# h3poteto/aws-global-accelerator-controller

Measured on NVIDIA H100. Metric: objects reconciled/sec at 10^6 Service+Ingress; change-set bit-exact vs Go ref, higher is better.
Workload: dtype u8/u32 (bytes and indices)

## Files before the change

### aws-global-accelerator-controller_b200/csrc/gar_engine.cu

```cuda

#include <cuda_runtime.h>
#include <unistd.h>

#include <cstdio>
#include <cstdlib>
#include <cstring>
#include <atomic>
#include <exception>
#include <functional>
#include <mutex>
#include <thread>
#include <string>
#include <vector>
#include <type_traits>
#include <utility>

#include "gar_pipeline.h"
#include "gar_shard.h"
#include "gar_delta.h"

#define GAR_VERSION_STRING "garecon 0.1.0 (sm_90a)"


template <class F>
// ... 97 lines not shown
template <class... Fs>
struct FPack;
template <>
struct FPack<> {
  __device__ __forceinline__ void call(int, u32) const {}
};
template <class F, class... R>
struct FPack<F, R...> {
  F f;
  FPack<R...> rest;
  FPack(const F &f_, const R &...r) : f(f_), rest(r...) {}
  __device__ __forceinline__ void call(int k, u32 i) const {
    if (k == 0) f(i);
    else rest.call(k - 1, i);
  }
};
constexpr int MULTI_MAX = 8;
struct MultiRanges {
  u32 blk_end[MULTI_MAX], n[MULTI_MAX];
  int count;
};
template <class P>
__global__ void __launch_bounds__(256) k_for_each_multi(const __grid_constant__ P pack, const __grid_constant__ MultiRanges r) {
  int k = 0;
  while (k + 1 < r.count && blockIdx.x >= r.blk_end[k]) k++;
  u32 i = (blockIdx.x - (k ? r.blk_end[k - 1] : 0u)) * blockDim.x + threadIdx.x;
  if (i < r.n[k]) pack.call(k, i);
}

template <class F> struct MinBlocks { static constexpr int value = 2; };
template <> struct MinBlocks<FGaObj> { static constexpr int value = 4; };
template <> struct MinBlocks<FR53Pair> { static constexpr int value = 6; };
template <> struct MinBlocks<FR53Prepare> { static constexpr int value = 6; };

__global__ void k_fill32(u32 *p, u32 v, size_t n) {
  size_t i = (size_t)blockIdx.x * blockDim.x + threadIdx.x;
  size_t stride = (size_t)gridDim.x * blockDim.x;
  for (; i < n; i += stride) p[i] = v;
}

constexpr int SCAN_THREADS = 256;
constexpr int SCAN_ITEMS = 8;
constexpr int SCAN_TILE = SCAN_THREADS * SCAN_ITEMS;

__device__ __forceinline__ u32 warp_incl_scan(u32 v) {
  const unsigned lane = threadIdx.x & 31;
#pragma unroll
  for (int d = 1; d < 32; d <<= 1) {
    u32 t = __shfl_up_sync(0xffffffffu, v, d);
    if (lane >= (unsigned)d) v += t;
  }
  return v;
}
__device__ __forceinline__ u32 block_excl_scan(u32 v, u32 *total) {
  __shared__ u32 wsum[SCAN_THREADS / 32];
  __shared__ u32 wtot;
  const unsigned lane = threadIdx.x & 31, w = threadIdx.x >> 5;
  u32 inc = warp_incl_scan(v);
  if (lane == 31) wsum[w] = inc;
  __syncthreads();
  if (w == 0) {
    u32 s = lane < SCAN_THREADS / 32 ? wsum[lane] : 0;
    u32 si = warp_incl_scan(s);
    if (lane < SCAN_THREADS / 32) wsum[lane] = si - s;
    if (lane == SCAN_THREADS / 32 - 1) wtot = si;
  }
// ... 1551 lines not shown
```

### aws-global-accelerator-controller_b200/csrc/gar_pipeline.h

```cpp
#pragma once

#include <stdio.h>
#include <stdlib.h>

#include <initializer_list>

#include "gar_rows.h"

#if defined(__CUDA_ARCH__)
#define GAR_ATOMIC_ADD(p, v) atomicAdd((p), (v))
#else
#define GAR_ATOMIC_ADD(p, v) (*(p) += (v))
#endif


enum Slot {
  S_DERIVED, S_OFLAGS, S_OKEY_HASH, S_STAGE_GA, S_STAGE_R53, S_ANN_R53, S_ANN_NAME, S_ANN_TAGS, S_ANN_LISTEN, S_DPORT_BEGIN, S_DPORTS,
  S_TOK_CODE, S_TOK_NAME, S_TOK_REGION,
  S_ACC_FLAGS, S_ACC_OWNER_KEY, S_ACC_OWNER, S_ACC_THOST, S_ACC_MANAGED, S_ACC_OWNER_HASH, S_ACC_THOST_HASH, S_REC_NAME_HASH, S_VAL_KEY_HASH,
  S_REC_ZONE, S_VAL_REC, S_VAL_CLS, S_VAL_KEY, S_VAL_ORPHAN, S_VAL_LINK, S_ACC_DIGEST,
  S_R53_MODE, S_R53_ACC, S_R53_ACC_DNS, S_PAIR_BEGIN, S_PAIR_OBJ, S_PAIR_HN, S_PAIR_CODE, S_PAIR_ZONE, S_PAIR_REC,
  S_IX_LB, S_IX_OWNER = S_IX_LB + 3, S_IX_THOST = S_IX_OWNER + 3, S_IX_ZONE = S_IX_THOST + 3, S_IX_VAL = S_IX_ZONE + 3,
  S_IX_ALIAS = S_IX_VAL + 3, S_IX_OBJ = S_IX_ALIAS + 3, S_IX_OVN = S_IX_OBJ + 3,
  S_SORT_KEYS = S_IX_OVN + 3, S_SORT_VALS, S_SORT_KEYS_ALT, S_SORT_VALS_ALT, S_SORT_TAGS,
  S_COUNTS, S_STATUS_GA, S_STATUS_R53, S_OPS, S_ERRFLAG, S_IX_EG, S_IX_EG_ENT, S_IX_EG_PAD,
  S_VAL_OBJ, S_ACC_OBJ, S_OBJ_CANON, S_OWN_BEGIN, S_OWN_FILL, S_OWN_ENT, S_OWN_MULTI,
  S_IXA_BEGIN, S_IXA_FILL, S_IXA_ENT, S_IXA_MULTI, S_OVN_FILL, S_OVN_MULTI, S_LB_HASH, S_REC_FLAGS,
  S_NSLOTS
};


struct FClassify {
  DevTables T;
  Work W;
  u32 *derived_public;
  u8 *oflags;
  u32 *errflag;
  GAR_HD void operator()(u32 i) const {
    classify_object(T, W, i);
    W.obj_canon[i] = i;
    u32 dv = W.derived[i];
    if (dv & OBJ_KEY_BAD) GAR_ATOMIC_ADD(errflag, 1u);
    derived_public[i] = dv & 0xFFu;
  }
};
struct FTokenise {
  DevTables T;
  Work W;
  static constexpr int kStageCols = 1;
  static constexpr u32 kStageBytes = 24 * 1024;
  static constexpr bool kStageByDefault = true;
  GAR_HD void operator()(u32 i) const { tokenise_hostname(T, W, i); }
  GAR_HD const u8 *stage_slab(int) const { return T.o.slab; }
  GAR_HD bool stage_window(int, u32 r0, u32 r1, u64 *lo, u64 *hi) const {
    gar_str a = T.o.lbi_hostname[r0], b = T.o.lbi_hostname[r1 - 1];
    *lo = GAR_STR_OFF(a);
    *hi = GAR_STR_OFF(b) + GAR_STR_LEN(b);
    return true;
  }
  template <class View>
  GAR_HD void run(u32 i, const View &view) const { tokenise_hostname_at(T, W, i, view(0, T.o.lbi_hostname[i])); }
};
struct FDigestAccel {
  DevTables T;
  Work W;
  GAR_HD void operator()(u32 i) const { digest_accelerator(T, W, i); }
};
struct FExpand {
  const u32 *begin;
  u32 nparents;
  u32 *parent_of;
  GAR_HD void operator()(u32 c) const {
    u32 lo = 0, hi = nparents;
    while (hi - lo > 1) {
      u32 mid = (lo + hi) >> 1;
      if (begin[mid] <= c) lo = mid;
      else hi = mid;
    }
    parent_of[c] = lo;
  }
};
constexpr u32 REC_INLINE_VALUES = 32;
constexpr u32 REC_HUGE_VALUES = 4096;
struct DirectView {
  const u8 *slab;
  GAR_HD Str operator()(int, gar_str r) const { return mkstr(slab, r); }
};
struct FPrepareRecord {
  DevTables T;
  Work W;
  u32 *big, *huge;
  static constexpr int kStageCols = 2;
  static constexpr u32 kStageBytes = 16 * 1024;
  static constexpr bool kStageByDefault = true;
  GAR_HD const u8 *stage_slab(int) const { return T.a.slab; }
  GAR_HD bool stage_window(int c, u32 r0, u32 r1, u64 *lo, u64 *hi) const {
    if (c == 0) {
      gar_str a = T.a.rec_name[r0], b = T.a.rec_name[r1 - 1];
      *lo = GAR_STR_OFF(a);
// ... 744 lines not shown
      be.for_each("idx_place", nrows, FIdxPlace{keys, cursor, tmp, ent, nb});
      be.for_each("idx_order", nb, FIdxOrder{begin, ent, overflow, canon});
    } else if (nrows) {
      u32 *keys2 = (u32 *)be.ensure(S_SORT_KEYS_ALT, sizeof(u32) * (size_t)(nrows + 1));
      u32 *vals2 = (u32 *)be.ensure(S_SORT_VALS_ALT, sizeof(u32) * (size_t)(nrows + 1));
      be.sort_pairs(keys, vals, keys2, vals2, nrows, ilog2(nb) + 1);
      be.for_each("idx_gather", nrows, FIdxGather{vals, begin + nb, tmp, ent});
      if (canon.canon) be.for_each("idx_order", nb, FIdxCanon{begin, ent, canon});
    }
    return HashIdx{begin, ent, nb - 1};
  }

  bool prepared = false;
  u64 n_dports = 0;
  u32 *errflag = nullptr;

  u32 acc_guest_from = 0xFFFFFFFFu;
  u32 sharded = 0;
  bool orphan_sweep = true;
  bool allow_empty_cache = false;

  void alloc_obj_work() {
    const u32 n = T.o.n_objects, nlbi = T.o.n_lbi;
    W.derived = (u32 *)be.ensure(S_DERIVED, 4 * (size_t)(n + 1));
    W.okey_hash = (u64 *)be.ensure(S_OKEY_HASH, 8 * (size_t)(n + 1));
    W.ann_r53 = (gar_str *)be.ensure(S_ANN_R53, 8 * (size_t)(n + 1));
    W.ann_name = (gar_str *)be.ensure(S_ANN_NAME, 8 * (size_t)(n + 1));
    W.ann_tags = (gar_str *)be.ensure(S_ANN_TAGS, 8 * (size_t)(n + 1));
    W.ann_listen = (gar_str *)be.ensure(S_ANN_LISTEN, 8 * (size_t)(n + 1));
    W.dport_begin = (u32 *)be.out_dport_begin(n);
    W.tok_code = (u8 *)be.out_tok_code(nlbi);
    W.tok_name = (gar_str *)be.out_tok_name(nlbi);
    W.tok_region = (gar_str *)be.out_tok_region(nlbi);
    W.r53_mode = (u8 *)be.ensure(S_R53_MODE, (size_t)n + 1);
    W.r53_acc = (u32 *)be.ensure(S_R53_ACC, 4 * (size_t)(n + 1));
    W.r53_acc_dns = (gar_str *)be.ensure(S_R53_ACC_DNS, 8 * (size_t)(n + 1));
    W.obj_canon = (u32 *)be.ensure(S_OBJ_CANON, 4 * (size_t)(n + 1));
  }
  CanonHook canon_hook(u32 b0, u32 b1) const { return CanonHook{W.obj_canon, T.o.slab, b0, b1}; }
  void alloc_work() {
    const u32 nacc = T.a.n_accels, nrec = T.a.n_records, nval = T.a.n_values;
    alloc_obj_work();
    W.acc_flags = (u32 *)be.ensure(S_ACC_FLAGS, 4 * (size_t)(nacc + 1));
    W.acc_owner_key = (gar_str *)be.ensure(S_ACC_OWNER_KEY, 8 * (size_t)(nacc + 1));
    W.acc_owner = (gar_str *)be.ensure(S_ACC_OWNER, 8 * (size_t)(nacc + 1));
    W.acc_thost = (gar_str *)be.ensure(S_ACC_THOST, 8 * (size_t)(nacc + 1));
    W.acc_managed = (gar_str *)be.ensure(S_ACC_MANAGED, 8 * (size_t)(nacc + 1));
    W.acc_owner_hash = (u64 *)be.ensure(S_ACC_OWNER_HASH, 8 * (size_t)(nacc + 1));
    W.acc_thost_hash = (u64 *)be.ensure(S_ACC_THOST_HASH, 8 * (size_t)(nacc + 1));
    W.rec_name_hash = (u64 *)be.ensure(S_REC_NAME_HASH, 8 * (size_t)(nrec + 1));
    W.val_key_hash = (u64 *)be.ensure(S_VAL_KEY_HASH, 8 * (size_t)(nval + 1));
    W.rec_zone = (u32 *)be.ensure(S_REC_ZONE, 4 * (size_t)(nrec + 1));
    W.val_rec = (u32 *)be.ensure(S_VAL_REC, 4 * (size_t)(nval + 1));
    W.val_cls = (u8 *)be.ensure(S_VAL_CLS, nval + 1);
    W.val_key = (gar_str *)be.ensure(S_VAL_KEY, 8 * (size_t)(nval + 1));
    W.val_orphan = (u8 *)be.ensure(S_VAL_ORPHAN, nval + 1);
    W.val_obj = (u32 *)be.ensure(S_VAL_OBJ, 4 * (size_t)(nval + 1));
    W.acc_obj = (u32 *)be.ensure(S_ACC_OBJ, 4 * (size_t)(nacc + 1));
    W.val_link = (ValLink *)be.ensure(S_VAL_LINK, sizeof(ValLink) * (size_t)(nval + 1));
    W.acc_digest = (AccDigest *)be.ensure(S_ACC_DIGEST, sizeof(AccDigest) * (size_t)(nacc + 1));
    W.lb_hash = (u64 *)be.ensure(S_LB_HASH, 8 * (size_t)(T.a.n_lbs + 1));
    W.rec_flags = (u8 *)be.ensure(S_REC_FLAGS, (size_t)nrec + 1);
    for (int k = 0; k < IX_N; k++) W.hist[k] = IxHist{nullptr, 0};
    W.pair_cap = 0;
    W.dport_cap = 0;
    errflag = (u32 *)be.ensure(S_ERRFLAG, 256);
// ... 144 lines not shown
    arm_group_a(1u << IX_ALIAS);
    stage1();
    finish_group_a();
  }
  void prepare_directory() {
    alloc_work();
    arm_group_a((1u << IX_LB) | (1u << IX_THOST));
    if (T.o.n_lbi) be.for_each("tokenise_hostnames", T.o.n_lbi, FTokenise{T, W});
    if (T.a.n_accels) be.for_each("digest_accelerators", T.a.n_accels, FDigestAccel{T, W});
    if (T.a.n_lbs) be.for_each("hash_load_balancers", T.a.n_lbs, FLbHash{T, W});
    finish_group_a();
  }

  u32 dport_cap = 0, pair_cap = 0;
  u64 ops_cap = 0;
  bool tiny_caps = false;
  int prepare() {
    const u32 n = T.o.n_objects, nacc = T.a.n_accels, nzone = T.a.n_zones, nrec = T.a.n_records;
    alloc_work();
    if (!force_radix) arm_group_a((1u << IX_LB) | (1u << IX_THOST) | (1u << IX_ZONE) | (1u << IX_ALIAS) | (1u << IX_OBJ));
    stage1();
    listen_ports();

    u32 *overflow = errflag + FW_IDX_OVERFLOW;
    if (!force_radix) {
      finish_group_a();
    } else {
      W.ix_lb = build_index(S_IX_LB, T.a.n_lbs, 1, FRowLb{T, W}, overflow, true);
      W.ix_thost = build_index(S_IX_THOST, nacc, 1, FRowThost{T, W}, overflow, true);
      W.ix_zone = build_index(S_IX_ZONE, nzone, 1, FRowZone{T}, overflow, true);
      W.ix_alias = build_index(S_IX_ALIAS, nrec, 2, FRowAlias{T, W}, overflow, true);
      W.ix_obj = build_index(S_IX_OBJ, n, 1, FRowObj{T, W}, overflow, true, canon_hook(0, 0xFFFFFFFFu));
    }
    resolve_owners(true);
    obj_stale = false;
    owner_indexes = false;
    return GAR_OK;
  }
  void listen_ports() {
    const u32 n = T.o.n_objects;
    be.fill32(W.dport_begin, 0, (size_t)n + 1);
    if (n) be.for_each("listen_ports_count", n, FJsonCount{T, W});
    be.exclusive_scan(W.dport_begin, n + 1);
    be.for_each("gather_header", 1, FGatherHeader{W.dport_begin + n, errflag});
    if (dport_cap < n / 2 + 1024 && !(tiny_caps && dport_cap)) dport_cap = tiny_caps ? 1 : n / 2 + 1024;
    W.dport_cap = dport_cap;
    W.dports = (i32 *)be.out_dports(dport_cap);
    if (n) be.for_each("listen_ports_write", n, FJsonWrite{T, W});
  }

  bool obj_stale = false, owners_stale = false;
  void prepare_objects() {
    const u32 n = T.o.n_objects, nlbi = T.o.n_lbi;
    alloc_obj_work();
    be.fill32(errflag, 0, FW_WORDS);
    W.hist[IX_OBJ] = IxHist{nullptr, 0};
    u32 *derived_public = (u32 *)be.out_derived(n);
    if (n) be.for_each("classify_objects", n, FClassify{T, W, derived_public, nullptr, errflag});
    if (nlbi) be.for_each_staged("tokenise_hostnames", nlbi, FTokenise{T, W});
    listen_ports();
    W.ix_obj = build_index(S_IX_OBJ, n, 1, FRowObj{T, W}, errflag + FW_IDX_OVERFLOW, force_radix, canon_hook(0, 0xFFFFFFFFu));
    obj_stale = false;
    owners_stale = true;
  }
  int index_objects() {
    for (int attempt = 0; attempt < 2; attempt++) {
      if (!prepared) prepare();
      else if (obj_stale) prepare_objects();
      prepared = true;
      u32 fl[FW_WORDS];
      be.download(fl, errflag, sizeof(fl));
      if (fl[FW_BAD_KEYS]) return GAR_E_INVALID;
      if (fl[FW_IDX_OVERFLOW] && !force_radix) {
        force_radix = true;
        prepared = false;
        continue;
      }
      return GAR_OK;
    }
    return GAR_E_STATE;
  }

  u64 n_pairs = 0;
  void r53_relational(u32 slots, const u32 *rows, u32 *st_r53) {
    W.pair_begin = (u32 *)be.ensure(S_PAIR_BEGIN, 4 * (size_t)(slots + 2));
    be.fill32(W.pair_begin, 0, (size_t)slots + 1);
    if (slots) be.for_each_warp("r53_prepare", slots, FR53Prepare{T, W, st_r53, rows});
    be.exclusive_scan(W.pair_begin, slots + 1);
    if (pair_cap < slots + slots / 2 + 1024 && !(tiny_caps && pair_cap)) pair_cap = tiny_caps ? 1 : slots + slots / 2 + 1024;
    W.pair_cap = pair_cap;
    W.pair_obj = (u32 *)be.ensure(S_PAIR_OBJ, 4 * (size_t)(pair_cap + 1));
    W.pair_hn = (gar_str *)be.ensure(S_PAIR_HN, 8 * (size_t)(pair_cap + 1));
// ... 157 lines not shown
```

### aws-global-accelerator-controller_b200/csrc/gar_rows.h

```cpp
#pragma once

#include "gar_common.h"
#include "gar_json.h"


struct DevTables {
  gar_objects o;
  gar_actual a;
  const u8 *cluster;
  u32 cluster_len;
};

enum {
  OBJ_HAS_NAME_ANN = 1u << 8,
  OBJ_HAS_TAGS_ANN = 1u << 9,
  OBJ_KEY_BAD = 1u << 10,
};

enum {
  ACC_MINE = 1u << 0,
  ACC_OWNER_KEYED = 1u << 1,
  ACC_OWNER_INGRESS = 1u << 2,
  ACC_OWNER_3PART = 1u << 3,
  ACC_HAS_MANAGED = 1u << 4, ACC_HAS_OWNER = 1u << 5, ACC_HAS_THOST = 1u << 6,
// ... 3 lines not shown
  R53_MODE_DONE = 0,
  R53_MODE_PAIRS = 1,
  R53_MODE_OBJECT = 2,
};
enum { PAIR_IN_SYNC = 0, PAIR_CREATE = 1, PAIR_UPSERT = 2, PAIR_NO_ZONE = 3,
       PAIR_REPEAT = 4 };
#define VALNAME_HAS_BACKSLASH (1u << 30)

enum { VAL_NOT_OWNER = 0, VAL_OWNER_SERVICE = 1, VAL_OWNER_INGRESS = 2, VAL_OWNER_3PART = 4 };

struct alignas(64) AccDigest {
  u32 flags;
  u32 lis;
  u32 eg;
  u32 pr_begin;
  u32 ep_begin;
  u16 n_ports, n_eps;
  i32 port0, port1;
  gar_str name;
  gar_str thost;
  gar_str owner_key;
  gar_str ep0;
};
enum {
  ACCD_ENABLED = 1u << 8,
  ACCD_MANAGED_TRUE = 1u << 9,
  ACCD_LIS_NONE = 1u << 10, ACCD_LIS_MANY = 1u << 11,
  ACCD_LIS_UDP = 1u << 12,
  ACCD_EG_NONE = 1u << 13, ACCD_EG_MANY = 1u << 14,
};
struct alignas(16) ValLink {
  u32 alias_row, pad;
  gar_str alias_dns;
};

enum IxId { IX_LB, IX_OWNER, IX_THOST, IX_ZONE, IX_VAL, IX_ALIAS, IX_OBJ, IX_OVN, IX_N };
struct IxHist {
  u32 *cnt;
  u32 mask;
};
#if defined(__CUDA_ARCH__)
#define GAR_HIST_ADD(p) atomicAdd((p), 1u)
#else
#define GAR_HIST_ADD(p) (++*(p))
#endif
GAR_HD void ix_count(const IxHist &h, u64 key_hash) {
  if (h.cnt) GAR_HIST_ADD(&h.cnt[(u32)key_hash & h.mask]);
}

struct Work {
  IxHist hist[IX_N];
  u64 *lb_hash;
  u8 *rec_flags;
  u32 pair_cap;
  u32 dport_cap;
  u32 *derived;
  u64 *okey_hash;
  gar_str *ann_r53;
  gar_str *ann_name;
  gar_str *ann_tags;
  gar_str *ann_listen;
  u32 *dport_begin;
  i32 *dports;
  u8 *tok_code;
  gar_str *tok_name, *tok_region;
  u32 *acc_flags;
  gar_str *acc_owner_key;
  gar_str *acc_owner;
  gar_str *acc_thost;
  gar_str *acc_managed;
  AccDigest *acc_digest;
  u64 *acc_owner_hash;
  u64 *acc_thost_hash;
  u32 *rec_zone;
  u64 *rec_name_hash;
  u32 *val_rec;
  u8 *val_cls;
  gar_str *val_key;
  u64 *val_key_hash;
  u8 *val_orphan;
  ValLink *val_link;
  u32 acc_guest_from;
  u32 sharded;
  u32 *val_obj;
  u32 *acc_obj;
  u32 *obj_canon;
  u32 *own_begin;
  const IdxEntry *own;
  u8 *r53_mode;
  u32 *r53_acc;
  gar_str *r53_acc_dns;
  u32 *pair_begin;
  u32 *pair_obj;
  gar_str *pair_hn;
  u8 *pair_code;
  u32 *pair_zone;
  u32 *pair_rec;
  HashIdx ix_lb;
// ... 410 lines not shown
  Cursor c = u_open(W.ix_lb, active, h);
  u32 found = GAR_NONE;
  U_BUCKET_LOOP(found == GAR_NONE, c) {
    IdxEntry e;
    bool hit = u_bucket_step(W.ix_lb, found == GAR_NONE, c, &e);
    bool eq = u_streq(hit, mkstr(T.a.slab, e.s0), name);
    eq = u_streq(eq, mkstr(T.a.slab, e.s1), region);
    if (eq) {
      found = e.row;
      *state = e.a0;
    }
  }
  return found;
}

GAR_HD u32 u_find_by_hostname(const DevTables &T, const Work &W, bool active, Str hostname, u32 *first, gar_str *first_dns) {
  Cursor c = u_open(W.ix_thost, active, u_hash(active, hostname));
  u32 n = 0;
  *first = GAR_NONE;
  U_BUCKET_LOOP(n < 2, c) {
    IdxEntry e;
    bool hit = u_bucket_step(W.ix_thost, n < 2, c, &e);
    if (u_streq(hit, mkstr(T.a.slab, e.s0), hostname)) {
      if (n == 0) {
        *first = e.row;
        *first_dns = e.s1;
      }
      n++;
    }
  }
  return n;
}

GAR_HD u32 u_find_hosted_zone(const DevTables &T, const Work &W, bool active, Str hostname) {
  Str t = hostname;
  u32 zone = GAR_NONE;
  bool walking = active;
  for (;;) {
    bool round = walking && t.n != 0;
    if (!GAR_ANY(round)) break;
    bool probe = round && zone_len_possible(W, t.n);
    Cursor c = u_open(W.ix_zone, probe, u_hash(probe, t));
    U_BUCKET_LOOP(zone == GAR_NONE, c) {
      IdxEntry e;
      bool hit = u_bucket_step(W.ix_zone, zone == GAR_NONE, c, &e);
      Str zn = mkstr(T.a.slab, e.s0);
      hit = hit && zn.n == t.n + 1;
      if (u_streq(hit, substr(zn, 0, hit ? t.n : 0), t)) zone = e.row;
    }
    u32 k = u_find_byte(round && zone == GAR_NONE, t, 0, '.');
    if (round) {
      if (zone != GAR_NONE || k >= t.n) walking = false;
      else t = substr(t, k + 1, t.n - k - 1);
    }
  }
  return zone;
}

GAR_HD u32 u_first_alias_a(const DevTables &T, const Work &W, bool active, u32 zone, Str name, gar_str *alias_dns) {
  Cursor c = u_open(W.ix_alias, active, hmix((u64)zone + 0x100, u_hash(active, name)));
  u32 found = GAR_NONE;
  U_BUCKET_LOOP(found == GAR_NONE, c) {
    IdxEntry e;
    bool hit = u_bucket_step(W.ix_alias, found == GAR_NONE, c, &e);
    hit = hit && e.a0 == zone && e.a1 == GAR_RR_A;
    if (u_streq(hit, mkstr(T.a.slab, e.s0), name)) {
// ... 222 lines not shown
  const gar_actual &A = T.a;
  u32 result = GAR_STATUS(GAR_ST_IGNORED, 0, 0);
  u32 dv = 0, kind = 0, jb = 0, nj = 0;
  Str okey{T.o.slab, 0};
  bool ensure = false;
  if (valid) {
    dv = W.derived[i];
    if (dv & GAR_DV_GA_ELIGIBLE) {
      jb = o.obj_lbi_begin[i];
      nj = o.obj_lbi_begin[i + 1] - jb;
      kind = o.obj_kind[i];
      if (nj < 1) {
        result = GAR_STATUS(GAR_ST_SKIP_NO_LB, 0, 0);
      } else {
        okey = object_key(T, i);
        if (!(dv & GAR_DV_GA_MANAGED)) {
          const OwnRange ar = own_accs(W, i);
          for (u32 p = ar.pos; p < ar.end; p++) put_delete_chain(T, s, i, kind, W.own[p].row);
          result = GAR_STATUS(GAR_ST_OK, 0, GAR_EV_DELETED);
        } else {
          ensure = true;
        }
      }
    }
  }
  u32 ev = 0;
  bool stop = false;
  u32 prev_lb = GAR_NONE;
  bool pending = false;
  for (u32 j = 0;; j++) {
    bool act = ensure && !stop && j < nj;
    if (!GAR_ANY(act)) break;
    bool probe = false;
    Str hostname{o.slab, 0}, tregion{o.slab, 0}, tname{o.slab, 0};
    if (act) {
      u32 code = W.tok_code[jb + j];
      if (code == GAR_TOK_PANIC) {
        result = GAR_STATUS(GAR_ST_PANIC, 0, ev);
        stop = true;
      } else if (code == GAR_TOK_NOT_AWS) {
      } else if (code >= GAR_TOK_ERR_NOT_ELB) {
        result = GAR_STATUS(GAR_ST_ERR_RETRY, GAR_D_NOT_ELB + (code - GAR_TOK_ERR_NOT_ELB), ev);
        stop = true;
      } else {
        probe = true;
        hostname = mkstr(o.slab, o.lbi_hostname[jb + j]);
        tregion = mkstr(o.slab, W.tok_region[jb + j]);
        tname = mkstr(o.slab, W.tok_name[jb + j]);
      }
    }
    u32 lb_state = 0;
    u32 lb = u_find_lb(T, W, probe, tregion, tname, &lb_state);
    bool have_lb = probe && lb != GAR_NONE;
    Str lb_dns = have_lb ? mkstr(A.slab, A.lb_dns[lb]) : Str{A.slab, 0};
    bool dns_eq = u_streq(have_lb, lb_dns, hostname);
    bool go = false;
    if (probe) {
      if (!have_lb) {
        result = GAR_STATUS(GAR_ST_ERR_RETRY, GAR_D_LB_NOT_FOUND, ev);
        stop = true;
      } else if (!dns_eq) {
        result = GAR_STATUS(GAR_ST_ERR_RETRY, GAR_D_LB_DNS_MISMATCH, ev);
        stop = true;
      } else if (lb_state != GAR_LB_ACTIVE) {
        result = GAR_STATUS(GAR_ST_REQUEUE_30S, 0, ev);
        stop = true;
      } else {
        go = true;
      }
    }
    const bool later = go && prev_lb != GAR_NONE;
    if (later) ga_later_step(T, W, i, kind, okey, jb, j, lb, prev_lb, pending, s, &ev);
    go = go && !later;
    OwnRange oc = go ? own_accs(W, i) : OwnRange{0, 0};
    Str lb_arn = go ? mkstr(A.slab, A.lb_arn[lb]) : Str{A.slab, 0};
    u32 nacc = 0;
    for (;;) {
      bool a = go && !stop && oc.pos < oc.end;
      if (!GAR_ANY(a)) break;
      u32 acc = a ? W.own[oc.pos++].row : GAR_NONE;
      if (a) nacc++;
      AccDigest d;
      d.flags = 0;
      if (a) d = W.acc_digest[acc];
      if (u_accelerator_changed(T, W, a, i, dv, kind, acc, d, okey, lb_dns)) s.put(GAR_OP_HEAD(GAR_OP_GA_UPDATE_ACCEL, GAR_CTRL_GA, kind), i, j, acc, lb, GAR_NONE);
      u32 eg = GAR_NONE;
      if (a) {
        if (d.flags & ACCD_LIS_MANY) {
          result = GAR_STATUS(GAR_ST_ERR_RETRY, GAR_D_TOO_MANY_LISTENERS, ev);
          stop = true;
        } else if (d.flags & ACCD_LIS_NONE) {
          s.put(GAR_OP_HEAD(GAR_OP_GA_CREATE_LISTENER, GAR_CTRL_GA, kind), i, j, acc, GAR_NONE, GAR_NONE);
          s.put(GAR_OP_HEAD(GAR_OP_GA_CREATE_EG, GAR_CTRL_GA, kind), i, j, acc, GAR_NONE, lb);
        } else {
          u32 lis = d.lis;
          bool want_udp = kind == GAR_KIND_SERVICE && (dv & GAR_DV_PROTO_UDP);
          bool changed = ((d.flags & ACCD_LIS_UDP) != 0) != want_udp;
          if (!changed) {
            PortList want = desired_ports(T, W, i);
            if (d.n_ports <= 2 && want.n == d.n_ports && (d.n_ports < 1 || want.p[0] == d.port0) && (d.n_ports < 2 || (want.p[1] == d.port1 && d.port0 != d.port1))) changed = false;
            else changed = ports_changed(PortList{A.pr_from + d.pr_begin, d.n_ports == 0xFFFF ? A.lis_pr_begin[lis + 1] - d.pr_begin : d.n_ports}, want);
          }
          if (changed) s.put(GAR_OP_HEAD(GAR_OP_GA_UPDATE_LISTENER, GAR_CTRL_GA, kind), i, j, acc, lis, GAR_NONE);
          if (d.flags & ACCD_EG_MANY) {
            result = GAR_STATUS(GAR_ST_ERR_RETRY, GAR_D_TOO_MANY_EGS, ev);
            stop = true;
          } else if (d.flags & ACCD_EG_NONE) {
            s.put(GAR_OP_HEAD(GAR_OP_GA_CREATE_EG, GAR_CTRL_GA, kind), i, j, acc, lis, lb);
// ... 18 lines not shown
      pending = true;
    }
    if ((go || later) && !stop) prev_lb = lb;
  }
  if (ensure && !stop) result = GAR_STATUS(GAR_ST_OK, 0, ev);
  return result;
}

GAR_HD void ga_later_step(const DevTables &T, const Work &W, u32 i, u32 kind, Str okey, u32 jb, u32 j, u32 lb, u32 prev_lb, bool pending, OpSink &s, u32 *ev) {
  const gar_actual &A = T.a;
  bool keep_visible, user_thost;
  user_tag_effects(T, W, i, kind, okey, &keep_visible, &user_thost);
  if (!keep_visible) {
    s.put(GAR_OP_HEAD(GAR_OP_GA_CREATE_CHAIN, GAR_CTRL_GA, kind), i, j, lb, GAR_NONE, GAR_NONE);
    *ev |= GAR_EV_CREATED;
    return;
  }
  Str lb_arn = mkstr(A.slab, A.lb_arn[lb]);
  const bool dns_differs = !user_thost && !streq(mkstr(A.slab, A.lb_dns[lb]), mkstr(A.slab, A.lb_dns[prev_lb]));
  const bool arn_differs = !streq(lb_arn, mkstr(A.slab, A.lb_arn[prev_lb]));
  if (pending) {
    if (dns_differs) s.put(GAR_OP_HEAD(GAR_OP_GA_UPDATE_ACCEL, GAR_CTRL_GA, kind), i, j, GAR_PENDING, lb, GAR_NONE);
    if (arn_differs) s.put(GAR_OP_HEAD(GAR_OP_GA_UPDATE_EG, GAR_CTRL_GA, kind), i, j, GAR_PENDING, GAR_PENDING, lb);
  }
  const OwnRange ar = own_accs(W, i);
  for (u32 p = ar.pos; p < ar.end; p++) {
    const u32 acc = W.own[p].row;
    if (dns_differs) s.put(GAR_OP_HEAD(GAR_OP_GA_UPDATE_ACCEL, GAR_CTRL_GA, kind), i, j, acc, lb, GAR_NONE);
    const AccDigest d = W.acc_digest[acc];
    const bool created = (d.flags & (ACCD_LIS_NONE | ACCD_EG_NONE)) != 0;
    bool replaced = created;
    for (u32 jp = 0; jp < j && !replaced; jp++) {
      if (W.tok_code[jb + jp] > GAR_TOK_NLB) continue;
      u32 st;
      u32 lbp = find_lb(T, W, mkstr(T.o.slab, W.tok_region[jb + jp]), mkstr(T.o.slab, W.tok_name[jb + jp]), &st);
      if (lbp != GAR_NONE && !eg_contains(T, d, mkstr(A.slab, A.lb_arn[lbp]))) replaced = true;
    }
    const bool contains = replaced ? !arn_differs : eg_contains(T, d, lb_arn);
    if (!contains) s.put(GAR_OP_HEAD(GAR_OP_GA_UPDATE_EG, GAR_CTRL_GA, kind), i, j, acc, created ? GAR_PENDING : d.eg, lb);
  }
}


struct OwnedHit {
  u32 v, rec, zone;
  gar_str name;
};
GAR_HD OwnedHit owned_hit(const IdxEntry &e) { return OwnedHit{e.row, e.a0, e.a1 & 0x3FFFFFFFu, e.s1}; }
struct OwnedList {
  const IdxEntry *e;
  u32 n;
};
GAR_HD OwnedList owned_list(const Work &W, u32 i) {
  const OwnRange r = own_vals(W, i);
  return OwnedList{W.own + r.pos, r.end - r.pos};
}
GAR_HD OwnedHit owned_get(const DevTables &, const Work &, const OwnedList &o, u32 k) { return owned_hit(load_entry(o.e + k)); }
constexpr u32 OWNED_CACHE = 8;
struct Owned {
  OwnedHit hit[OWNED_CACHE];
  u32 n;
  u64 okh;
  u32 kind;
  Str key;
};
GAR_HD bool owned_match(const DevTables &T, const IdxEntry &e, u32 kind, Str key) {
  return (e.a1 >> 31) == kind && streq(mkstr(T.a.slab, e.s0), key);
}
// ... 92 lines not shown
}

GAR_HD u32 r53_reconcile(const DevTables &T, const Work &W, u32 i, bool valid, OpSink &s) {
  const gar_objects &o = T.o;
  const gar_actual &A = T.a;
  u32 result = GAR_STATUS(GAR_ST_IGNORED, 0, 0);
  u32 kind = 0, jb = 0, nj = 0;
  Str hostnames{T.o.slab, 0};
  bool ensure = false;
  OwnedList ow{W.own, 0};
  if (valid) {
    u32 dv = W.derived[i];
    if (dv & GAR_DV_R53_ELIGIBLE) {
      kind = o.obj_kind[i];
      if (!(dv & GAR_DV_R53_ANNOTATED)) {
        r53_cleanup(T, W, i, kind, owned_list(W, i), s);
        result = GAR_STATUS(GAR_ST_OK, 0, GAR_EV_DELETED);
      } else {
        ensure = true;
        hostnames = mkstr(o.slab, W.ann_r53[i]);
        jb = o.obj_lbi_begin[i];
        nj = o.obj_lbi_begin[i + 1] - jb;
      }
    }
  }
  u32 ev = 0;
  bool stop = false;
  bool have_prev = false;
  Str prev_acc_dns{A.slab, 0};
  for (u32 j = 0;; j++) {
    bool act = ensure && !stop && j < nj;
    if (!GAR_ANY(act)) break;
    bool probe = false;
    Str lbhost{o.slab, 0};
    if (act) {
      u32 code = W.tok_code[jb + j];
      if (code == GAR_TOK_PANIC) {
        result = GAR_STATUS(GAR_ST_PANIC, 0, ev);
        stop = true;
      } else if (code == GAR_TOK_NOT_AWS) {
      } else if (code >= GAR_TOK_ERR_NOT_ELB) {
        result = GAR_STATUS(GAR_ST_ERR_RETRY, GAR_D_NOT_ELB + (code - GAR_TOK_ERR_NOT_ELB), ev);
        stop = true;
      } else {
        probe = true;
        lbhost = mkstr(o.slab, o.lbi_hostname[jb + j]);
      }
    }
    u32 acc = GAR_NONE;
    gar_str acc_dns_ref = 0;
    u32 nacc = u_find_by_hostname(T, W, probe, lbhost, &acc, &acc_dns_ref);
    bool go = false;
    if (probe) {
      if (nacc > 1) {
        result = GAR_STATUS(GAR_ST_REQUEUE_60S, GAR_D_ACCEL_MANY, ev);
        stop = true;
      } else if (nacc == 0) {
        result = GAR_STATUS(GAR_ST_REQUEUE_60S, GAR_D_ACCEL_NONE, ev);
        stop = true;
      } else {
        go = true;
      }
    }
    Str acc_dns = go ? mkstr(A.slab, acc_dns_ref) : Str{A.slab, 0};
    if (go) ow = owned_list(W, i);
    bool created = false;
    u32 pos = 0, k = 0;
    for (;;) {
      bool more = go && !stop && pos <= hostnames.n;
      if (!GAR_ANY(more)) break;
      u32 comma = u_find_byte(more, hostnames, pos, ',');
      Str hn = more ? substr(hostnames, pos, comma - pos) : Str{o.slab, 0};
      pos = comma + 1;
      u32 zone = u_find_hosted_zone(T, W, more, hn);
      if (more && zone == GAR_NONE) {
        result = GAR_STATUS(GAR_ST_ERR_RETRY, GAR_D_NO_HOSTED_ZONE, ev);
        stop = true;
        more = false;
      }
      u32 rec = GAR_NONE;
      gar_str rec_alias = 0;
      for (u32 x = 0;; x++) {
        bool has = more && x < ow.n;
        if (!GAR_ANY(has)) break;
// ... 30 lines not shown
          }
        }
        k++;
      }
    }
    if (go && !stop && created) ev |= GAR_EV_CREATED;
    if (go && !stop) {
      have_prev = true;
      prev_acc_dns = acc_dns;
    }
  }
  if (ensure && !stop) result = GAR_STATUS(GAR_ST_OK, 0, ev);
  return result;
}


GAR_HD void link_value_alias(const DevTables &T, const Work &W, u32 v) {
  u32 row = GAR_NONE;
  gar_str dns = 0;
  if (W.val_cls[v] != VAL_NOT_OWNER) {
    u32 rec = W.val_rec[v];
    row = first_alias_a(T, W, W.rec_zone[rec], mkstr(T.a.slab, T.a.rec_name[rec]), W.rec_name_hash[rec], &dns);
  }
  ValLink l;
  l.alias_row = row;
  l.pad = 0;
  l.alias_dns = dns;
  W.val_link[v] = l;
}

GAR_HD void r53_prepare(const DevTables &T, const Work &W, u32 i, u32 t, bool valid, u32 *status) {
  const gar_objects &o = T.o;
  u32 mode = R53_MODE_DONE, st = GAR_STATUS(GAR_ST_IGNORED, 0, 0), npairs = 0;
  bool probe = false;
  Str lbhost{o.slab, 0}, hostnames{o.slab, 0};
  if (valid) {
    u32 dv = W.derived[i];
    if (dv & GAR_DV_R53_ELIGIBLE) {
      u32 jb = o.obj_lbi_begin[i], nj = o.obj_lbi_begin[i + 1] - jb;
      if (!(dv & GAR_DV_R53_ANNOTATED) || nj > 1) {
        mode = R53_MODE_OBJECT;
      } else if (nj == 0) {
        st = GAR_STATUS(GAR_ST_OK, 0, 0);
      } else {
        u32 code = W.tok_code[jb];
        if (code == GAR_TOK_PANIC) st = GAR_STATUS(GAR_ST_PANIC, 0, 0);
        else if (code == GAR_TOK_NOT_AWS) st = GAR_STATUS(GAR_ST_OK, 0, 0);
        else if (code >= GAR_TOK_ERR_NOT_ELB) st = GAR_STATUS(GAR_ST_ERR_RETRY, GAR_D_NOT_ELB + (code - GAR_TOK_ERR_NOT_ELB), 0);
        else {
          probe = true;
          lbhost = mkstr(o.slab, o.lbi_hostname[jb]);
          hostnames = mkstr(o.slab, W.ann_r53[i]);
        }
      }
    }
  }
  u32 acc = GAR_NONE;
  gar_str acc_dns = 0;
  u32 nacc = u_find_by_hostname(T, W, probe, lbhost, &acc, &acc_dns);
  bool go = false;
  if (probe) {
    if (nacc > 1) st = GAR_STATUS(GAR_ST_REQUEUE_60S, GAR_D_ACCEL_MANY, 0);
    else if (nacc == 0) st = GAR_STATUS(GAR_ST_REQUEUE_60S, GAR_D_ACCEL_NONE, 0);
    else go = true;
  }
  u32 pos = 0;
  for (;;) {
    bool more = go && pos <= hostnames.n;
    if (!GAR_ANY(more)) break;
    u32 comma = u_find_byte(more, hostnames, pos, ',');
    if (more) {
      npairs++;
      pos = comma + 1;
    }
  }
  if (go) mode = R53_MODE_PAIRS;
  if (valid) {
    W.r53_mode[i] = (u8)mode;
    W.r53_acc[i] = acc;
    W.r53_acc_dns[i] = acc_dns;
    W.pair_begin[t] = npairs;
    if (mode == R53_MODE_DONE) status[t] = st;
  }
}

GAR_HD void r53_fill_pairs(const DevTables &T, const Work &W, u32 i, u32 t) {
  if (W.r53_mode[i] != R53_MODE_PAIRS) return;
  gar_str ref = W.ann_r53[i];
  Str hostnames = mkstr(T.o.slab, ref);
  u32 p = W.pair_begin[t], pos = 0, np = 0;
  u32 st[8], ln[8];
  Str piece;
// ... 162 lines not shown
        break;
      }
    }
    if (dup) continue;
    s.put(GAR_OP_HEAD(GAR_OP_R53_DELETE_RECORD, GAR_CTRL_R53, 0), GAR_NONE, 0, zone, r, e.row);
  }
}


struct DevBindings {
  gar_bindings b;
  HashIdx ix_eg;
};

GAR_HD bool egb_eg_exists(const DevBindings &B, Str arn) {
  Cursor c = idx_open(B.ix_eg, gar_hash(arn));
  IdxEntry e;
  while (idx_next(B.ix_eg, c, &e))
    if (streq(mkstr(B.b.slab, e.s0), arn)) return true;
  return false;
}

GAR_HD u32 egb_lb_of(const DevTables &T, const Work &W, u32 lbi_row, u32 *detail) {
  u32 code = W.tok_code[lbi_row];
  *detail = 0;
  if (code == GAR_TOK_NOT_AWS || code == GAR_TOK_PANIC) {
    *detail = GAR_D_NOT_ELB;
    return GAR_NONE;
  }
  if (code >= GAR_TOK_ERR_NOT_ELB) {
    *detail = GAR_D_NOT_ELB + (code - GAR_TOK_ERR_NOT_ELB);
    return GAR_NONE;
  }
  u32 st;
  u32 lb = find_lb(T, W, mkstr(T.o.slab, W.tok_region[lbi_row]), mkstr(T.o.slab, W.tok_name[lbi_row]), &st);
  if (lb == GAR_NONE) *detail = GAR_D_LB_NOT_FOUND;
  return lb;
}

GAR_HD u32 egb_reconcile(const DevTables &T, const Work &W, const DevBindings &B, u32 k, OpSink &s) {
  const gar_bindings &b = B.b;
  const gar_actual &A = T.a;
  u32 flags = b.egb_flags[k];
  u32 eb = b.egb_ep_begin[k], n = b.egb_ep_begin[k + 1] - eb;
  Str eg_arn = mkstr(b.slab, b.egb_eg_arn[k]);
  auto H = [](u32 op) { return GAR_OP_HEAD(op, GAR_CTRL_EGB, 0); };
  if (flags & GAR_EGB_DELETING) {
    if (n == 0 || !egb_eg_exists(B, eg_arn)) {
      s.put(H(GAR_OP_EGB_REMOVE_FINALIZER), k, 0, GAR_NONE, GAR_NONE, GAR_NONE);
      return GAR_STATUS(GAR_ST_OK, 0, 0);
    }
    u32 len = n;
    for (u32 i = 0; i < n; i++) {
      u32 src = 2 * i < n - 1 ? 2 * i : n - 1;
      s.put(H(GAR_OP_EGB_REMOVE_ENDPOINT), k, 0, eb + src, GAR_NONE, GAR_NONE);
      if (i + 1 > len) return GAR_STATUS(GAR_ST_PANIC, 0, 0);
      len--;
    }
    s.put(H(GAR_OP_EGB_UPDATE_STATUS), k, 0, GAR_NONE, GAR_NONE, GAR_NONE);
    return GAR_STATUS(GAR_ST_REQUEUE_1S, 0, 0);
  }
  if (!(flags & GAR_EGB_HAS_FINALIZERS)) {
    s.put(H(GAR_OP_EGB_ADD_FINALIZER), k, 0, GAR_NONE, GAR_NONE, GAR_NONE);
    return GAR_STATUS(GAR_ST_OK, 0, 0);
  }
  u32 jb = 0, nj = 0;
  u32 refkind = b.egb_ref_kind[k];
  if (refkind != GAR_EGB_REF_NONE) {
// ... 69 lines not shown
```

Before: 181.1 million.

## Precompute per-LB-ingress join of load balancer and accelerator lookups

Adds a warp-cooperative pre-pass that, for each load-balancer ingress row, resolves the LB by region/name, checks DNS equality and state, and finds the matching accelerator by hostname. The results go into a new per-row LbiJoin table. GA reconcile, R53 reconcile, R53 prepare, the replaced-EG check and the EGB LB lookup now read this table instead of repeating the hash-index probes and string compares. This removes duplicated lookups across stages at the cost of an extra kernel and a 32-byte-per-row buffer. It also relies on the table being rebuilt whenever tokens or indexes change.

```diff
diff --git a/aws-global-accelerator-controller_b200/csrc/gar_engine.cu b/aws-global-accelerator-controller_b200/csrc/gar_engine.cu
--- a/aws-global-accelerator-controller_b200/csrc/gar_engine.cu
+++ b/aws-global-accelerator-controller_b200/csrc/gar_engine.cu
@@ -153,6 +153,7 @@
 template <> struct MinBlocks<FGaObj> { static constexpr int value = 4; };
 template <> struct MinBlocks<FR53Pair> { static constexpr int value = 6; };
 template <> struct MinBlocks<FR53Prepare> { static constexpr int value = 6; };
+template <> struct MinBlocks<FLbiJoin> { static constexpr int value = 6; };
 
 __global__ void k_fill32(u32 *p, u32 v, size_t n) {
   size_t i = (size_t)blockIdx.x * blockDim.x + threadIdx.x;
diff --git a/aws-global-accelerator-controller_b200/csrc/gar_pipeline.h b/aws-global-accelerator-controller_b200/csrc/gar_pipeline.h
--- a/aws-global-accelerator-controller_b200/csrc/gar_pipeline.h
+++ b/aws-global-accelerator-controller_b200/csrc/gar_pipeline.h
@@ -25,7 +25,7 @@
   S_SORT_KEYS = S_IX_OVN + 3, S_SORT_VALS, S_SORT_KEYS_ALT, S_SORT_VALS_ALT, S_SORT_TAGS,
   S_COUNTS, S_STATUS_GA, S_STATUS_R53, S_OPS, S_ERRFLAG, S_IX_EG, S_IX_EG_ENT, S_IX_EG_PAD,
   S_VAL_OBJ, S_ACC_OBJ, S_OBJ_CANON, S_OWN_BEGIN, S_OWN_FILL, S_OWN_ENT, S_OWN_MULTI,
-  S_IXA_BEGIN, S_IXA_FILL, S_IXA_ENT, S_IXA_MULTI, S_OVN_FILL, S_OVN_MULTI, S_LB_HASH, S_REC_FLAGS,
+  S_IXA_BEGIN, S_IXA_FILL, S_IXA_ENT, S_IXA_MULTI, S_OVN_FILL, S_OVN_MULTI, S_LB_HASH, S_REC_FLAGS, S_LBI_JOIN,
   S_NSLOTS
 };
 
@@ -65,6 +65,11 @@
   DevTables T;
   Work W;
   GAR_HD void operator()(u32 i) const { digest_accelerator(T, W, i); }
+};
+struct FLbiJoin {
+  DevTables T;
+  Work W;
+  GAR_HD void operator()(u32 l, bool valid) const { lbi_join(T, W, l, valid); }
 };
 struct FExpand {
   const u32 *begin;
@@ -875,6 +880,7 @@
     W.tok_code = (u8 *)be.out_tok_code(nlbi);
     W.tok_name = (gar_str *)be.out_tok_name(nlbi);
     W.tok_region = (gar_str *)be.out_tok_region(nlbi);
+    W.lbi_join = (LbiJoin *)be.ensure(S_LBI_JOIN, sizeof(LbiJoin) * (size_t)(nlbi + 1));
     W.r53_mode = (u8 *)be.ensure(S_R53_MODE, (size_t)n + 1);
     W.r53_acc = (u32 *)be.ensure(S_R53_ACC, 4 * (size_t)(n + 1));
     W.r53_acc_dns = (gar_str *)be.ensure(S_R53_ACC_DNS, 8 * (size_t)(n + 1));
@@ -1085,10 +1091,14 @@
       W.ix_alias = build_index(S_IX_ALIAS, nrec, 2, FRowAlias{T, W}, overflow, true);
       W.ix_obj = build_index(S_IX_OBJ, n, 1, FRowObj{T, W}, overflow, true, canon_hook(0, 0xFFFFFFFFu));
     }
+    lbi_joins();
     resolve_owners(true);
     obj_stale = false;
     owner_indexes = false;
     return GAR_OK;
+  }
+  void lbi_joins() {
+    if (T.o.n_lbi) be.for_each_warp("lbi_joins", T.o.n_lbi, FLbiJoin{T, W});
   }
   void listen_ports() {
     const u32 n = T.o.n_objects;
@@ -1111,6 +1121,7 @@
     u32 *derived_public = (u32 *)be.out_derived(n);
     if (n) be.for_each("classify_objects", n, FClassify{T, W, derived_public, nullptr, errflag});
     if (nlbi) be.for_each_staged("tokenise_hostnames", nlbi, FTokenise{T, W});
+    lbi_joins();
     listen_ports();
     W.ix_obj = build_index(S_IX_OBJ, n, 1, FRowObj{T, W}, errflag + FW_IDX_OVERFLOW, force_radix, canon_hook(0, 0xFFFFFFFFu));
     obj_stale = false;
diff --git a/aws-global-accelerator-controller_b200/csrc/gar_rows.h b/aws-global-accelerator-controller_b200/csrc/gar_rows.h
--- a/aws-global-accelerator-controller_b200/csrc/gar_rows.h
+++ b/aws-global-accelerator-controller_b200/csrc/gar_rows.h
@@ -59,6 +59,16 @@
 struct alignas(16) ValLink {
   u32 alias_row, pad;
   gar_str alias_dns;
+};
+enum { LBI_LB_NOT_FOUND = 0, LBI_LB_DNS_MISMATCH = 1, LBI_LB_NOT_ACTIVE = 2, LBI_LB_OK = 3 };
+struct alignas(32) LbiJoin {
+  u32 lb;
+  u32 acc;
+  gar_str arn;
+  gar_str acc_dns;
+  u8 outcome;
+  u8 nacc;
+  u8 pad[6];
 };
 
 enum IxId { IX_LB, IX_OWNER, IX_THOST, IX_ZONE, IX_VAL, IX_ALIAS, IX_OBJ, IX_OVN, IX_N };
@@ -91,6 +101,7 @@
   i32 *dports;
   u8 *tok_code;
   gar_str *tok_name, *tok_region;
+  LbiJoin *lbi_join;
   u32 *acc_flags;
   gar_str *acc_owner_key;
   gar_str *acc_owner;
@@ -567,6 +578,30 @@
   return n;
 }
 
+GAR_HD void lbi_join(const DevTables &T, const Work &W, u32 row, bool valid) {
+  const bool probe = valid && W.tok_code[row] <= GAR_TOK_NLB;
+  Str host{T.o.slab, 0}, region{T.o.slab, 0}, name{T.o.slab, 0};
+  if (probe) {
+    host = mkstr(T.o.slab, T.o.lbi_hostname[row]);
+    region = mkstr(T.o.slab, W.tok_region[row]);
+    name = mkstr(T.o.slab, W.tok_name[row]);
+  }
+  u32 state = 0;
+  const u32 lb = u_find_lb(T, W, probe, region, name, &state);
+  const bool have_lb = probe && lb != GAR_NONE;
+  const bool dns_eq = u_streq(have_lb, have_lb ? mkstr(T.a.slab, T.a.lb_dns[lb]) : Str{T.a.slab, 0}, host);
+  LbiJoin r;
+  r.acc_dns = 0;
+  const u32 nacc = u_find_by_hostname(T, W, probe, host, &r.acc, &r.acc_dns);
+  if (!probe) return;
+  r.lb = lb;
+  r.arn = have_lb ? T.a.lb_arn[lb] : 0;
+  r.outcome = !have_lb ? LBI_LB_NOT_FOUND : !dns_eq ? LBI_LB_DNS_MISMATCH : state != GAR_LB_ACTIVE ? LBI_LB_NOT_ACTIVE : LBI_LB_OK;
+  r.nacc = (u8)nacc;
+  for (int k = 0; k < 6; k++) r.pad[k] = 0;
+  W.lbi_join[row] = r;
+}
+
 GAR_HD u32 u_find_hosted_zone(const DevTables &T, const Work &W, bool active, Str hostname) {
   Str t = hostname;
   u32 zone = GAR_NONE;
@@ -855,7 +890,6 @@
     bool act = ensure && !stop && j < nj;
     if (!GAR_ANY(act)) break;
     bool probe = false;
-    Str hostname{o.slab, 0}, tregion{o.slab, 0}, tname{o.slab, 0};
     if (act) {
       u32 code = W.tok_code[jb + j];
       if (code == GAR_TOK_PANIC) {
@@ -867,25 +901,21 @@
         stop = true;
       } else {
         probe = true;
-        hostname = mkstr(o.slab, o.lbi_hostname[jb + j]);
-        tregion = mkstr(o.slab, W.tok_region[jb + j]);
-        tname = mkstr(o.slab, W.tok_name[jb + j]);
-      }
-    }
-    u32 lb_state = 0;
-    u32 lb = u_find_lb(T, W, probe, tregion, tname, &lb_state);
-    bool have_lb = probe && lb != GAR_NONE;
-    Str lb_dns = have_lb ? mkstr(A.slab, A.lb_dns[lb]) : Str{A.slab, 0};
-    bool dns_eq = u_streq(have_lb, lb_dns, hostname);
+      }
+    }
+    u32 lb = GAR_NONE;
     bool go = false;
     if (probe) {
-      if (!have_lb) {
+      const LbiJoin *jr = W.lbi_join + jb + j;
+      lb = jr->lb;
+      const u32 outcome = jr->outcome;
+      if (outcome == LBI_LB_NOT_FOUND) {
         result = GAR_STATUS(GAR_ST_ERR_RETRY, GAR_D_LB_NOT_FOUND, ev);
         stop = true;
-      } else if (!dns_eq) {
+      } else if (outcome == LBI_LB_DNS_MISMATCH) {
         result = GAR_STATUS(GAR_ST_ERR_RETRY, GAR_D_LB_DNS_MISMATCH, ev);
         stop = true;
-      } else if (lb_state != GAR_LB_ACTIVE) {
+      } else if (outcome == LBI_LB_NOT_ACTIVE) {
         result = GAR_STATUS(GAR_ST_REQUEUE_30S, 0, ev);
         stop = true;
       } else {
@@ -896,7 +926,8 @@
     if (later) ga_later_step(T, W, i, kind, okey, jb, j, lb, prev_lb, pending, s, &ev);
     go = go && !later;
     OwnRange oc = go ? own_accs(W, i) : OwnRange{0, 0};
-    Str lb_arn = go ? mkstr(A.slab, A.lb_arn[lb]) : Str{A.slab, 0};
+    Str lb_dns = go ? mkstr(o.slab, o.lbi_hostname[jb + j]) : Str{o.slab, 0};
+    Str lb_arn = go ? mkstr(A.slab, W.lbi_join[jb + j].arn) : Str{A.slab, 0};
     u32 nacc = 0;
     for (;;) {
       bool a = go && !stop && oc.pos < oc.end;
@@ -981,8 +1012,7 @@
     bool replaced = created;
     for (u32 jp = 0; jp < j && !replaced; jp++) {
       if (W.tok_code[jb + jp] > GAR_TOK_NLB) continue;
-      u32 st;
-      u32 lbp = find_lb(T, W, mkstr(T.o.slab, W.tok_region[jb + jp]), mkstr(T.o.slab, W.tok_name[jb + jp]), &st);
+      const u32 lbp = W.lbi_join[jb + jp].lb;
       if (lbp != GAR_NONE && !eg_contains(T, d, mkstr(A.slab, A.lb_arn[lbp]))) replaced = true;
     }
     const bool contains = replaced ? !arn_differs : eg_contains(T, d, lb_arn);
@@ -1141,7 +1171,6 @@
     bool act = ensure && !stop && j < nj;
     if (!GAR_ANY(act)) break;
     bool probe = false;
-    Str lbhost{o.slab, 0};
     if (act) {
       u32 code = W.tok_code[jb + j];
       if (code == GAR_TOK_PANIC) {
@@ -1153,12 +1182,16 @@
         stop = true;
       } else {
         probe = true;
-        lbhost = mkstr(o.slab, o.lbi_hostname[jb + j]);
-      }
-    }
-    u32 acc = GAR_NONE;
+      }
+    }
+    u32 acc = GAR_NONE, nacc = 0;
     gar_str acc_dns_ref = 0;
-    u32 nacc = u_find_by_hostname(T, W, probe, lbhost, &acc, &acc_dns_ref);
+    if (probe) {
+      const LbiJoin *jr = W.lbi_join + jb + j;
+      nacc = jr->nacc;
+      acc = jr->acc;
+      acc_dns_ref = jr->acc_dns;
+    }
     bool go = false;
     if (probe) {
       if (nacc > 1) {
@@ -1255,8 +1288,10 @@
 GAR_HD void r53_prepare(const DevTables &T, const Work &W, u32 i, u32 t, bool valid, u32 *status) {
   const gar_objects &o = T.o;
   u32 mode = R53_MODE_DONE, st = GAR_STATUS(GAR_ST_IGNORED, 0, 0), npairs = 0;
+  u32 acc = GAR_NONE, nacc = 0;
+  gar_str acc_dns = 0;
   bool probe = false;
-  Str lbhost{o.slab, 0}, hostnames{o.slab, 0};
+  Str hostnames{o.slab, 0};
   if (valid) {
     u32 dv = W.derived[i];
     if (dv & GAR_DV_R53_ELIGIBLE) {
@@ -1272,15 +1307,15 @@
         else if (code >= GAR_TOK_ERR_NOT_ELB) st = GAR_STATUS(GAR_ST_ERR_RETRY, GAR_D_NOT_ELB + (code - GAR_TOK_ERR_NOT_ELB), 0);
         else {
           probe = true;
-          lbhost = mkstr(o.slab, o.lbi_hostname[jb]);
           hostnames = mkstr(o.slab, W.ann_r53[i]);
+          const LbiJoin *jr = W.lbi_join + jb;
+          nacc = jr->nacc;
+          acc = jr->acc;
+          acc_dns = jr->acc_dns;
         }
       }
     }
   }
-  u32 acc = GAR_NONE;
-  gar_str acc_dns = 0;
-  u32 nacc = u_find_by_hostname(T, W, probe, lbhost, &acc, &acc_dns);
   bool go = false;
   if (probe) {
     if (nacc > 1) st = GAR_STATUS(GAR_ST_REQUEUE_60S, GAR_D_ACCEL_MANY, 0);
@@ -1509,8 +1544,7 @@
     *detail = GAR_D_NOT_ELB + (code - GAR_TOK_ERR_NOT_ELB);
     return GAR_NONE;
   }
-  u32 st;
-  u32 lb = find_lb(T, W, mkstr(T.o.slab, W.tok_region[lbi_row]), mkstr(T.o.slab, W.tok_name[lbi_row]), &st);
+  const u32 lb = W.lbi_join[lbi_row].lb;
   if (lb == GAR_NONE) *detail = GAR_D_LB_NOT_FOUND;
   return lb;
 }
```

Result: faster. 183.5 million, median of 6 (+1.3%).
